# Guitaricet/relora

Measured on NVIDIA H100. Metric: training throughput, llama ReLoRA (tokens/s, whole job, device-timed, max over ranks), higher is better.
Workload: dtype bf16

## Files before the change

relora_b200/csrc/attention.cu:

```cuda
#include <cuda.h>

#include <cstdio>
#include <cstdlib>
#include <mutex>
#include <stdexcept>
#include <string>
#include <unordered_map>

#include "attention.h"
#include "common.cuh"
#include "sm90.cuh"
#include "tensormap.h"

namespace rb {

using namespace sm90;

namespace {

constexpr int BQ = 64;
constexpr int kPanel = 64 * 128;
constexpr int kThreads = 128;
constexpr int kMaxHeadDim = 256;
constexpr float kNegInf = -1e30f;

constexpr int smem_bytes(int nres, int np) { return (nres + 4) * np * kPanel + 1024 + 1024; }
constexpr int dq_out_panels(int np) { return np <= 3 ? np : 2; }
constexpr int dkv_out_panels(int np) { return np <= 2 ? np : 2; }
constexpr int splits(int np, int no) { return (np + no - 1) / no; }

__device__ __forceinline__ float fast_exp2(float x) {
  float y;
  asm("ex2.approx.ftz.f32 %0, %1;" : "=f"(y) : "f"(x));
  return y;
}

__device__ __forceinline__ void frag_to_a(const float (&d)[32], int kk, uint32_t (&a)[4]) {
  a[0] = pack_bf16x2(d[8 * kk + 0], d[8 * kk + 1]);
  a[1] = pack_bf16x2(d[8 * kk + 2], d[8 * kk + 3]);
  a[2] = pack_bf16x2(d[8 * kk + 4], d[8 * kk + 5]);
  a[3] = pack_bf16x2(d[8 * kk + 6], d[8 * kk + 7]);
}
template <int NSTEPS>
__device__ __forceinline__ void mma_steps_kk(float (&d)[32], uint32_t a, uint32_t b) {
#pragma unroll
  for (int ks = 0; ks < NSTEPS; ++ks) {
    const uint32_t ofs = (ks >> 2) * kPanel + (ks & 3) * 32;
    wgmma_bf16_ss_n64<0, 0>(d, desc_kmajor(a + ofs), desc_kmajor(b + ofs));
  }
}
template <int NP>
__device__ __forceinline__ void mma_tiles_kk(float (&d)[32], uint32_t a, uint32_t b, int nks) {
  if constexpr (NP == 1) {
    mma_steps_kk<4>(d, a, b);
  } else {
    switch (nks - 4 * (NP - 1)) {
      case 1: mma_steps_kk<4 * NP - 3>(d, a, b); break;
      case 2: mma_steps_kk<4 * NP - 2>(d, a, b); break;
      case 3: mma_steps_kk<4 * NP - 1>(d, a, b); break;
      default: mma_steps_kk<4 * NP>(d, a, b); break;
    }
  }
}
__device__ __forceinline__ void pack_a(const float (&p)[32], uint32_t (&a)[4][4]) {
#pragma unroll
  for (int kk = 0; kk < 4; ++kk) {
    frag_to_a(p, kk, a[kk]);
    fence_regs(a[kk]);
  }
}
template <int NO, int N = NO>
__device__ __forceinline__ void mma_regs_tile(float (&d)[NO][32], const uint32_t (&a)[4][4], uint32_t t, int nout) {
  if constexpr (N > 1) {
    if (nout < N) return mma_regs_tile<NO, N - 1>(d, a, t, nout);
  }
#pragma unroll
  for (int kk = 0; kk < 4; ++kk) {
#pragma unroll
    for (int j = 0; j < N; ++j) wgmma_bf16_rs_n64<1>(d[j], a[kk], desc_mnmajor(t + j * kPanel + kk * 2048));
  }
}
__device__ __forceinline__ void zero32(float (&d)[32]) {
#pragma unroll
  for (int i = 0; i < 32; ++i) d[i] = 0.f;
}

struct Smem {
  uint8_t* res[2];
  uint8_t* str[2][2];
  uint64_t* res_bar;
  uint64_t* str_bar;
  float* col_lse;
  float* col_delta;
};
template <int NRES, int NP>
__device__ __forceinline__ Smem smem_layout() {
  constexpr int kTile = NP * kPanel;
  extern __shared__ uint8_t smem_raw[];
  uint8_t* s = reinterpret_cast<uint8_t*>((reinterpret_cast<uintptr_t>(smem_raw) + 1023) & ~uintptr_t(1023));
  Smem m;
  m.res[0] = s;
  m.res[1] = s + (NRES - 1) * kTile;
  for (int b = 0; b < 2; ++b)
    for (int o = 0; o < 2; ++o) m.str[b][o] = s + (NRES + 2 * b + o) * kTile;
  m.res_bar = reinterpret_cast<uint64_t*>(s + (NRES + 4) * kTile);
  m.str_bar = m.res_bar + 1;
  m.col_lse = reinterpret_cast<float*>(s + (NRES + 4) * kTile + 64);
  m.col_delta = m.col_lse + 64;
  return m;
}
struct TileSrc {
  const CUtensorMap* map;
  int head;
};
template <int NP>
__device__ __forceinline__ void load_tile(TileSrc s, uint64_t* bar, uint8_t* dst, int row) {
#pragma unroll
  for (int pn = 0; pn < NP; ++pn) tma_load_3d(s.map, bar, dst + pn * kPanel, 64 * pn, s.head, row);
}
template <int NP>
__device__ __forceinline__ void issue_pair(const Smem& m, int buf, TileSrc s0, TileSrc s1, int row) {
  mbar_arrive_expect_tx(&m.str_bar[buf], 2 * NP * kPanel);
  load_tile<NP>(s0, &m.str_bar[buf], m.str[buf][0], row);
  load_tile<NP>(s1, &m.str_bar[buf], m.str[buf][1], row);
}
template <int NRES, int NP>
__device__ __forceinline__ void prologue(const Smem& m, TileSrc r0, TileSrc r1, int res_row, TileSrc s0, TileSrc s1, int row0, int nblk) {
  if (threadIdx.x == 0) {
    mbar_init(m.res_bar, 1);
    mbar_init(&m.str_bar[0], 1);
    mbar_init(&m.str_bar[1], 1);
    fence_barrier_init();
  }
  __syncthreads();
  pdl_wait();
  if (warp_id() == 0) {
    if (elect_one()) {
      mbar_arrive_expect_tx(m.res_bar, NRES * NP * kPanel);
      load_tile<NP>(r0, m.res_bar, m.res[0], res_row);
      if (NRES == 2) load_tile<NP>(r1, m.res_bar, m.res[1], res_row);
      for (int j = 0; j < 2 && j < nblk; ++j) issue_pair<NP>(m, j, s0, s1, row0 + j * BQ);
    }
    __syncwarp();
  }
  mbar_wait(m.res_bar, 0);
}

struct HeadMap {
  int hs, wk, wv, group;
  __device__ __forceinline__ int q(int h) const { return h * hs; }
  __device__ __forceinline__ int k(int kv) const { return kv * hs + wk; }
  __device__ __forceinline__ int v(int kv) const { return kv * hs + wv; }
};
struct FwdArgs {
  bf16* out;
  long long ld_out;
  float* lse;
  int B, T, nh, hd;
  float scale_log2;
  HeadMap hm;
};

template <int NP>
__global__ void __launch_bounds__(kThreads) attn_fwd_kernel(const __grid_constant__ CUtensorMap map_qkv, const FwdArgs p) {
  if (threadIdx.x == 0) pdl_launch_dependents();
  const int nqb = (p.T + BQ - 1) / BQ;
  const int qb = nqb - 1 - blockIdx.x;
  const int h = blockIdx.y, b = blockIdx.z;
  const int q0 = qb * BQ, rowbase = b * p.T;
  const int nkb = qb + 1;
  const int nks = (p.hd + 15) / 16;
  const Smem m = smem_layout<1, NP>();
  const int kv = h / p.hm.group;
  const int hq = p.hm.q(h), hk = p.hm.k(kv), hv = p.hm.v(kv);
  prologue<1, NP>(m, {&map_qkv, hq}, {&map_qkv, hq}, rowbase + q0, {&map_qkv, hk}, {&map_qkv, hv}, rowbase, nkb);
  const uint32_t sq = smem_u32(m.res[0]);
  float o[NP][32], mrow[2] = {kNegInf, kNegInf}, lrow[2] = {0.f, 0.f};
#pragma unroll
  for (int pn = 0; pn < NP; ++pn) zero32(o[pn]);
  const int r_lo = q0 + frag_row(0);
  for (int j = 0; j < nkb; ++j) {
    const int buf = j & 1;
    mbar_wait(&m.str_bar[buf], (j >> 1) & 1);
    float s[32];
    zero32(s);
    wgmma_fence();
    mma_tiles_kk<NP>(s, sq, smem_u32(m.str[buf][0]), nks);
    wgmma_commit();
    wgmma_wait<0>();
    fence_regs(s);
    float mx[2] = {mrow[0], mrow[1]};
#pragma unroll
    for (int i = 0; i < 32; ++i) {
      const int hr = (i >> 1) & 1;
      float v = s[i] * p.scale_log2;
      if (j == qb && j * BQ + frag_col(i) > r_lo + 8 * hr) v = kNegInf;
      s[i] = v;
      mx[hr] = fmaxf(mx[hr], v);
    }
#pragma unroll
    for (int hr = 0; hr < 2; ++hr) {
      mx[hr] = fmaxf(mx[hr], __shfl_xor_sync(0xffffffffu, mx[hr], 1));
      mx[hr] = fmaxf(mx[hr], __shfl_xor_sync(0xffffffffu, mx[hr], 2));
    }
    const float corr[2] = {fast_exp2(mrow[0] - mx[0]), fast_exp2(mrow[1] - mx[1])};
    float ls[2] = {0.f, 0.f};
#pragma unroll
    for (int i = 0; i < 32; ++i) {
      const int hr = (i >> 1) & 1;
      s[i] = fast_exp2(s[i] - mx[hr]);
      ls[hr] += s[i];
#pragma unroll
      for (int pn = 0; pn < NP; ++pn) o[pn][i] *= corr[hr];
    }
#pragma unroll
    for (int hr = 0; hr < 2; ++hr) {
      lrow[hr] = lrow[hr] * corr[hr] + ls[hr];
      mrow[hr] = mx[hr];
    }
    uint32_t pa[4][4];
    pack_a(s, pa);
#pragma unroll
    for (int pn = 0; pn < NP; ++pn) fence_regs(o[pn]);
    wgmma_fence();
    mma_regs_tile<NP>(o, pa, smem_u32(m.str[buf][1]), NP);
    wgmma_commit();
    wgmma_wait<0>();
#pragma unroll
    for (int pn = 0; pn < NP; ++pn) fence_regs(o[pn]);
    __syncthreads();
    if (warp_id() == 0 && j + 2 < nkb) {
      if (elect_one()) issue_pair<NP>(m, buf, {&map_qkv, hk}, {&map_qkv, hv}, rowbase + (j + 2) * BQ);
      __syncwarp();
    }
  }
#pragma unroll
  for (int hr = 0; hr < 2; ++hr) {
    lrow[hr] += __shfl_xor_sync(0xffffffffu, lrow[hr], 1);
    lrow[hr] += __shfl_xor_sync(0xffffffffu, lrow[hr], 2);
  }
#pragma unroll
  for (int pn = 0; pn < NP; ++pn) {
#pragma unroll
    for (int i = 0; i < 32; i += 2) {
      const int hr = (i >> 1) & 1;
      const int q = r_lo + 8 * hr, c = 64 * pn + frag_col(i);
      if (q >= p.T || c >= p.hd) continue;
      const float inv = 1.f / lrow[hr];
      *reinterpret_cast<uint32_t*>(p.out + (long long)(rowbase + q) * p.ld_out + h * p.hd + c) =
          pack_bf16x2(o[pn][i] * inv, o[pn][i + 1] * inv);
    }
  }
  if ((threadIdx.x & 3) == 0) {
#pragma unroll
    for (int hr = 0; hr < 2; ++hr) {
      const int q = r_lo + 8 * hr;
      if (q < p.T) p.lse[((long long)b * p.nh + h) * p.T + q] = mrow[hr] + __log2f(lrow[hr]);
    }
  }
}

__global__ void __launch_bounds__(256) attn_delta_kernel(const bf16* __restrict__ o, long long ld_o, const bf16* __restrict__ dout,
                                                         long long ld_do, float* __restrict__ delta, int B, int T, int nh, int hd) {
  pdl_wait();
  pdl_launch_dependents();
  const long long total = (long long)B * T * nh;
  for (long long i = blockIdx.x * (long long)blockDim.x + threadIdx.x; i < total; i += (long long)gridDim.x * blockDim.x) {
    const int h = int(i % nh);
    const long long row = i / nh;
    const bf16* a = o + row * ld_o + h * hd;
    const bf16* g = dout + row * ld_do + h * hd;
    float acc = 0.f;
    for (int q = 0; q < hd; q += 8) {
      float x[8], y[8];
      unpack8(*reinterpret_cast<const uint4*>(a + q), x);
      unpack8(*reinterpret_cast<const uint4*>(g + q), y);
#pragma unroll
      for (int j = 0; j < 8; ++j) acc += x[j] * y[j];
    }
    const long long bb = row / T, t = row % T;
    delta[(bb * nh + h) * T + t] = acc;
  }
}

struct BwdArgs {
  const float* lse;
  const float* delta;
  bf16* dqkv;
  long long ld_dqkv;
  int B, T, nh, hd;
  float scale, scale_log2;
  HeadMap hm;
};

__device__ __forceinline__ void store_rows(bf16* base, long long ld, int row0, int rows_valid, int col_ofs, int hd, const float (&d)[32], float sc) {
#pragma unroll
  for (int i = 0; i < 32; i += 2) {
    const int r = frag_row(i), c = frag_col(i);
    if (row0 + r >= rows_valid || c >= hd) continue;
    *reinterpret_cast<uint32_t*>(base + (long long)row0 * ld + (long long)r * ld + col_ofs + c) = pack_bf16x2(d[i] * sc, d[i + 1] * sc);
  }
}
template <int NO>
__device__ __forceinline__ void store_panels(bf16* base, long long ld, int row0, int rows_valid, int col_ofs, int hd, int pn0, int nout,
                                             const float (&d)[NO][32], float sc) {
#pragma unroll
  for (int j = 0; j < NO; ++j)
    if (j < nout) store_rows(base, ld, row0, rows_valid, col_ofs + 64 * (pn0 + j), hd - 64 * (pn0 + j), d[j], sc);
}

template <int NP>
__global__ void __launch_bounds__(kThreads) attn_bwd_dq_kernel(const __grid_constant__ CUtensorMap map_qkv,
                                                               const __grid_constant__ CUtensorMap map_do, const BwdArgs p) {
  constexpr int NO = dq_out_panels(NP), NSPLIT = splits(NP, dq_out_panels(NP));
  if (threadIdx.x == 0) pdl_launch_dependents();
  const int nqb = (p.T + BQ - 1) / BQ;
  const int qb = nqb - 1 - blockIdx.x / NSPLIT;
  const int pn0 = (blockIdx.x % NSPLIT) * NO;
  const int nout = NP % NO == 0 ? NO : min(NO, NP - pn0);
  const int h = blockIdx.y, b = blockIdx.z;
  const int q0 = qb * BQ, rowbase = b * p.T;
  const int nkb = qb + 1;
  const int nks = (p.hd + 15) / 16;
  const Smem m = smem_layout<2, NP>();
  const int kv = h / p.hm.group;
  const int hq = p.hm.q(h), hk = p.hm.k(kv), hv = p.hm.v(kv);
  prologue<2, NP>(m, {&map_qkv, hq}, {&map_do, h}, rowbase + q0, {&map_qkv, hk}, {&map_qkv, hv}, rowbase, nkb);
  const long long bh = (long long)b * p.nh + h;
  const int r_lo = q0 + frag_row(0);
  float lse[2], dlt[2];
#pragma unroll
  for (int hr = 0; hr < 2; ++hr) {
    const int q = min(r_lo + 8 * hr, p.T - 1);
    lse[hr] = p.lse[bh * p.T + q];
    dlt[hr] = p.delta[bh * p.T + q];
  }
  float dq[NO][32];
#pragma unroll
  for (int j = 0; j < NO; ++j) zero32(dq[j]);
  for (int j = 0; j < nkb; ++j) {
    const int buf = j & 1;
    mbar_wait(&m.str_bar[buf], (j >> 1) & 1);
    float s[32], dp[32];
    zero32(s);
    zero32(dp);
    wgmma_fence();
    mma_tiles_kk<NP>(s, smem_u32(m.res[0]), smem_u32(m.str[buf][0]), nks);
    mma_tiles_kk<NP>(dp, smem_u32(m.res[1]), smem_u32(m.str[buf][1]), nks);
    wgmma_commit();
    wgmma_wait<0>();
    fence_regs(s);
    fence_regs(dp);
#pragma unroll
    for (int i = 0; i < 32; ++i) {
      const int hr = (i >> 1) & 1;
      const bool ok = !(j == qb && j * BQ + frag_col(i) > r_lo + 8 * hr);
      const float pr = ok ? fast_exp2(s[i] * p.scale_log2 - lse[hr]) : 0.f;
      s[i] = pr * (dp[i] - dlt[hr]);
    }
    uint32_t pa[4][4];
    pack_a(s, pa);
    wgmma_fence();
    mma_regs_tile<NO>(dq, pa, smem_u32(m.str[buf][0]) + pn0 * kPanel, nout);
    wgmma_commit();
    wgmma_wait<0>();
#pragma unroll
    for (int jo = 0; jo < NO; ++jo) fence_regs(dq[jo]);
    __syncthreads();
    if (warp_id() == 0 && j + 2 < nkb) {
      if (elect_one()) issue_pair<NP>(m, buf, {&map_qkv, hk}, {&map_qkv, hv}, rowbase + (j + 2) * BQ);
      __syncwarp();
    }
  }
  store_panels<NO>(p.dqkv + (long long)rowbase * p.ld_dqkv, p.ld_dqkv, q0, p.T, hq * p.hd, p.hd, pn0, nout, dq, p.scale);
}

template <int NP>
__global__ void __launch_bounds__(kThreads) attn_bwd_dkv_kernel(const __grid_constant__ CUtensorMap map_qkv,
                                                                const __grid_constant__ CUtensorMap map_do, const BwdArgs p) {
  constexpr int NO = dkv_out_panels(NP), NSPLIT = splits(NP, dkv_out_panels(NP));
  if (threadIdx.x == 0) pdl_launch_dependents();
  const int nkb = (p.T + BQ - 1) / BQ;
  const int kb = blockIdx.x / NSPLIT;
  const int pn0 = (blockIdx.x % NSPLIT) * NO;
  const int nout = NP % NO == 0 ? NO : min(NO, NP - pn0);
  const int kv = blockIdx.y, b = blockIdx.z;
  const int k0 = kb * BQ, rowbase = b * p.T;
  const int nblk = nkb - kb;
  const int nks = (p.hd + 15) / 16;
  const Smem m = smem_layout<2, NP>();
  const int h0 = kv * p.hm.group;
  prologue<2, NP>(m, {&map_qkv, p.hm.k(kv)}, {&map_qkv, p.hm.v(kv)}, rowbase + k0, {&map_qkv, p.hm.q(h0)}, {&map_do, h0}, rowbase + k0, nblk);
  if (nblk == 1 && p.hm.group > 1 && warp_id() == 0) {
    if (elect_one()) issue_pair<NP>(m, 1, {&map_qkv, p.hm.q(h0 + 1)}, {&map_do, h0 + 1}, rowbase + k0);
    __syncwarp();
  }
  const int key_lo = k0 + frag_row(0);
  float dk[NO][32], dv[NO][32];
#pragma unroll
  for (int j = 0; j < NO; ++j) {
    zero32(dk[j]);
    zero32(dv[j]);
  }
  int hg = h0, qs = k0;
  for (int jj = 0; hg < ((int)blockIdx.y + 1) * p.hm.group; ++jj) {
    const int buf = jj & 1;
    const long long bh = (long long)b * p.nh + hg;
    if (threadIdx.x < BQ) {
      const int qc = min(qs + (int)threadIdx.x, p.T - 1);
      m.col_lse[threadIdx.x] = p.lse[bh * p.T + qc];
      m.col_delta[threadIdx.x] = p.delta[bh * p.T + qc];
    }
    __syncthreads();
    mbar_wait(&m.str_bar[buf], (jj >> 1) & 1);
    float st[32], dpt[32];
    zero32(st);
    zero32(dpt);
    wgmma_fence();
    mma_tiles_kk<NP>(st, smem_u32(m.res[0]), smem_u32(m.str[buf][0]), nks);
    mma_tiles_kk<NP>(dpt, smem_u32(m.res[1]), smem_u32(m.str[buf][1]), nks);
    wgmma_commit();
    wgmma_wait<0>();
    fence_regs(st);
    fence_regs(dpt);
#pragma unroll
    for (int i = 0; i < 32; ++i) {
      const int q = qs + frag_col(i), key = key_lo + 8 * ((i >> 1) & 1);
      const bool ok = q < p.T && key <= q;
      const float pr = ok ? fast_exp2(st[i] * p.scale_log2 - m.col_lse[frag_col(i)]) : 0.f;
      dpt[i] = pr * (dpt[i] - m.col_delta[frag_col(i)]);
      st[i] = pr;
    }
    uint32_t pa[4][4], dsa[4][4];
    pack_a(st, pa);
    pack_a(dpt, dsa);
    wgmma_fence();
    mma_regs_tile<NO>(dv, pa, smem_u32(m.str[buf][1]) + pn0 * kPanel, nout);
    mma_regs_tile<NO>(dk, dsa, smem_u32(m.str[buf][0]) + pn0 * kPanel, nout);
    wgmma_commit();
    wgmma_wait<0>();
#pragma unroll
    for (int j = 0; j < NO; ++j) {
      fence_regs(dv[j]);
      fence_regs(dk[j]);
    }
    __syncthreads();
    if (warp_id() == 0) {
      int h2 = hg, q2 = qs + 2 * BQ;
      while (q2 >= p.T) {
        q2 -= nkb * BQ - k0;
        ++h2;
      }
      if (h2 < ((int)blockIdx.y + 1) * p.hm.group) {
        if (elect_one()) issue_pair<NP>(m, buf, {&map_qkv, p.hm.q(h2)}, {&map_do, h2}, rowbase + q2);
        __syncwarp();
      }
    }
    qs += BQ;
    if (qs >= p.T) {
      qs = k0;
      ++hg;
    }
  }
  bf16* base = p.dqkv + (long long)rowbase * p.ld_dqkv;
  store_panels<NO>(base, p.ld_dqkv, k0, p.T, p.hm.k(blockIdx.y) * p.hd, p.hd, pn0, nout, dk, p.scale);
  store_panels<NO>(base, p.ld_dqkv, k0, p.T, p.hm.v(blockIdx.y) * p.hd, p.hd, pn0, nout, dv, 1.0f);
}

struct HeadMapKey {
  const void* ptr;
  long long ld, rows;
  int hd, heads;
  bool operator==(const HeadMapKey& o) const { return ptr == o.ptr && ld == o.ld && rows == o.rows && hd == o.hd && heads == o.heads; }
};
struct HeadMapHash {
  size_t operator()(const HeadMapKey& k) const {
    size_t h = reinterpret_cast<size_t>(k.ptr);
    h ^= std::hash<long long>()(k.ld * 1315423911ll + k.rows) + 0x9e3779b97f4a7c15ull + (h << 6) + (h >> 2);
    h ^= std::hash<long long>()(((long long)k.hd << 32) | (unsigned)k.heads) + 0x9e3779b97f4a7c15ull + (h << 6) + (h >> 2);
    return h;
  }
};
std::unordered_map<HeadMapKey, CUtensorMap, HeadMapHash> g_head_maps;
std::mutex g_head_maps_mu;

CUtensorMap head_map(const void* ptr, long long ld, long long rows, int hd, int heads) {
  HeadMapKey key{ptr, ld, rows, hd, heads};
  {
    std::lock_guard<std::mutex> lk(g_head_maps_mu);
    auto it = g_head_maps.find(key);
    if (it != g_head_maps.end()) return it->second;
  }
  CUtensorMap m = make_map_3d_bf16(ptr, hd, heads, rows, hd, ld, 64, 1, 64);
  std::lock_guard<std::mutex> lk(g_head_maps_mu);
  if (g_head_maps.size() > 4096) g_head_maps.clear();
  g_head_maps.emplace(key, m);
  return m;
}

void check_shape(int B, int T, int nh, int nkv, int hd, bool interleaved) {
  if (B <= 0 || T <= 0 || nh <= 0) throw std::runtime_error("attention: empty problem");
  if (hd <= 0 || hd % 8 != 0 || hd > kMaxHeadDim)
    throw std::runtime_error("attention: head_dim must be a multiple of 8 and <= 256, got " + std::to_string(hd));
  if (nkv <= 0 || nh % nkv != 0)
    throw std::runtime_error("attention: nh (" + std::to_string(nh) + ") must be a multiple of nkv (" + std::to_string(nkv) + ")");
  if (interleaved && nkv != nh) throw std::runtime_error("attention: the interleaved qkv layout has no grouped-query form (nkv must equal nh)");
}

HeadMap head_map_of(int nh, int nkv, bool interleaved) {
  return interleaved ? HeadMap{3, 1, 2, 1} : HeadMap{1, nh, nh + nkv, nh / nkv};
}

template <int NP>
void fwd_np(const AttnDesc& d, const CUtensorMap& map, cudaStream_t stream) {
  constexpr int smem = smem_bytes(1, NP);
  static const bool configured =
      (check(cudaFuncSetAttribute(attn_fwd_kernel<NP>, cudaFuncAttributeMaxDynamicSharedMemorySize, smem), "cudaFuncSetAttribute(attn_fwd)"), true);
  (void)configured;
  FwdArgs p;
  p.out = reinterpret_cast<bf16*>(d.out); p.ld_out = d.ld_out; p.lse = d.lse;
  p.B = d.B; p.T = d.T; p.nh = d.nh; p.hd = d.hd;
  p.scale_log2 = d.scale * 1.4426950408889634f;
  p.hm = head_map_of(d.nh, d.nkv, d.interleaved);
  const dim3 grid((unsigned)((d.T + BQ - 1) / BQ), (unsigned)d.nh, (unsigned)d.B);
  launch_k(attn_fwd_kernel<NP>, grid, kThreads, smem, stream, map, p);
  RB_CHECK_LAUNCH("attn_fwd_kernel");
}

template <int NP>
void bwd_np(const AttnBwdDesc& d, const CUtensorMap& map_qkv, const CUtensorMap& map_do, cudaStream_t stream) {
  constexpr int smem = smem_bytes(2, NP);
  static const bool configured =
      (check(cudaFuncSetAttribute(attn_bwd_dq_kernel<NP>, cudaFuncAttributeMaxDynamicSharedMemorySize, smem), "cudaFuncSetAttribute(attn_dq)"),
       check(cudaFuncSetAttribute(attn_bwd_dkv_kernel<NP>, cudaFuncAttributeMaxDynamicSharedMemorySize, smem), "cudaFuncSetAttribute(attn_dkv)"),
       true);
  (void)configured;
  BwdArgs p;
  p.lse = d.lse; p.delta = d.delta; p.dqkv = reinterpret_cast<bf16*>(d.dqkv); p.ld_dqkv = d.ld_dqkv;
  p.B = d.B; p.T = d.T; p.nh = d.nh; p.hd = d.hd;
  p.scale = d.scale; p.scale_log2 = d.scale * 1.4426950408889634f;
  p.hm = head_map_of(d.nh, d.nkv, d.interleaved);
  const unsigned nblk = (unsigned)((d.T + BQ - 1) / BQ);
  const dim3 grid_dkv(nblk * splits(NP, dkv_out_panels(NP)), (unsigned)d.nkv, (unsigned)d.B);
  launch_k(attn_bwd_dkv_kernel<NP>, grid_dkv, kThreads, smem, stream, map_qkv, map_do, p);
  RB_CHECK_LAUNCH("attn_bwd_dkv_kernel");
  const dim3 grid_dq(nblk * splits(NP, dq_out_panels(NP)), (unsigned)d.nh, (unsigned)d.B);
  launch_k(attn_bwd_dq_kernel<NP>, grid_dq, kThreads, smem, stream, map_qkv, map_do, p);
  RB_CHECK_LAUNCH("attn_bwd_dq_kernel");
}

int panels(int hd) { return (hd + 63) / 64; }

}

void attention_fwd(const AttnDesc& d, cudaStream_t stream) {
  check_shape(d.B, d.T, d.nh, d.nkv, d.hd, d.interleaved);
  const long long rows = (long long)d.B * d.T;
  CUtensorMap map = head_map(d.qkv, d.ld_qkv, rows, d.hd, d.nh + 2 * d.nkv);
  switch (panels(d.hd)) {
    case 1: fwd_np<1>(d, map, stream); break;
    case 2: fwd_np<2>(d, map, stream); break;
    case 3: fwd_np<3>(d, map, stream); break;
    default: fwd_np<4>(d, map, stream); break;
  }
}

void attention_bwd(const AttnBwdDesc& d, cudaStream_t stream) {
  check_shape(d.B, d.T, d.nh, d.nkv, d.hd, d.interleaved);
  const long long rows = (long long)d.B * d.T;
  CUtensorMap map_qkv = head_map(d.qkv, d.ld_qkv, rows, d.hd, d.nh + 2 * d.nkv);
  CUtensorMap map_do = head_map(d.dout, d.ld_dout, rows, d.hd, d.nh);
  {
    const long long total = rows * d.nh;
    const int grid = (int)std::min<long long>((total + 255) / 256, (long long)num_sms() * 8);
    launch_k(attn_delta_kernel, grid, 256, 0, stream, reinterpret_cast<const bf16*>(d.out), d.ld_out, reinterpret_cast<const bf16*>(d.dout),
             d.ld_dout, d.delta, d.B, d.T, d.nh, d.hd);
    RB_CHECK_LAUNCH("attn_delta_kernel");
  }
  switch (panels(d.hd)) {
    case 1: bwd_np<1>(d, map_qkv, map_do, stream); break;
    case 2: bwd_np<2>(d, map_qkv, map_do, stream); break;
    case 3: bwd_np<3>(d, map_qkv, map_do, stream); break;
    default: bwd_np<4>(d, map_qkv, map_do, stream); break;
  }
}

int attention_smem_bytes(int hd) { return smem_bytes(2, panels(hd)); }

long long attention_ds_pitch(int T) { return ((long long)T + 63) / 64 * 64; }
long long attention_ds_workspace_elems(int B, int T, int nh) {
  const long long Tp = attention_ds_pitch(T);
  return (long long)B * nh * Tp * Tp;
}

}
```

Measured before the change: 215,100.

## Prefetch dKV backward LSE/delta stats via cp.async into double-buffered smem

The dK/dV backward kernel used to load per-query LSE and delta values with plain global loads plus a __syncthreads at the top of every iteration. Those loads now go through cp.async into a double-buffered stats region and are tied to the same mbarrier as the TMA tile loads. The barrier arrival count is raised to cover the 32 cp.async arrivals from warp 0. This removes a blocking global load and a full-block barrier from each loop step, at the cost of a little extra shared memory and more complex barrier accounting.

```diff
diff --git a/relora_b200/csrc/attention.cu b/relora_b200/csrc/attention.cu
--- a/relora_b200/csrc/attention.cu
+++ b/relora_b200/csrc/attention.cu
@@ -25,6 +25,7 @@
 constexpr float kNegInf = -1e30f;
 
 constexpr int smem_bytes(int nres, int np) { return (nres + 4) * np * kPanel + 1024 + 1024; }
+constexpr int kStatsBytes = 2 * 128 * 4;
 constexpr int dq_out_panels(int np) { return np <= 3 ? np : 2; }
 constexpr int dkv_out_panels(int np) { return np <= 2 ? np : 2; }
 constexpr int splits(int np, int no) { return (np + no - 1) / no; }
@@ -90,8 +91,7 @@
   uint8_t* str[2][2];
   uint64_t* res_bar;
   uint64_t* str_bar;
-  float* col_lse;
-  float* col_delta;
+  float* stats;
 };
 template <int NRES, int NP>
 __device__ __forceinline__ Smem smem_layout() {
@@ -105,8 +105,7 @@
     for (int o = 0; o < 2; ++o) m.str[b][o] = s + (NRES + 2 * b + o) * kTile;
   m.res_bar = reinterpret_cast<uint64_t*>(s + (NRES + 4) * kTile);
   m.str_bar = m.res_bar + 1;
-  m.col_lse = reinterpret_cast<float*>(s + (NRES + 4) * kTile + 64);
-  m.col_delta = m.col_lse + 64;
+  m.stats = reinterpret_cast<float*>(s + (NRES + 4) * kTile + 1024);
   return m;
 }
 struct TileSrc {
@@ -375,6 +374,36 @@
   store_panels<NO>(p.dqkv + (long long)rowbase * p.ld_dqkv, p.ld_dqkv, q0, p.T, hq * p.hd, p.hd, pn0, nout, dq, p.scale);
 }
 
+__device__ __forceinline__ void cp_async_4(void* smem_dst, const void* gmem_src) {
+  asm volatile("cp.async.ca.shared.global [%0], [%1], 4;" ::"r"(smem_u32(smem_dst)), "l"(gmem_src) : "memory");
+}
+__device__ __forceinline__ void cp_async_arrive_noinc(uint64_t* bar) {
+  asm volatile("cp.async.mbarrier.arrive.noinc.shared::cta.b64 [%0];" ::"r"(smem_u32(bar)) : "memory");
+}
+template <int NP>
+__device__ __forceinline__ void dkv_issue(const Smem& m, int buf, const CUtensorMap* map_qkv, const CUtensorMap* map_do,
+                                          const BwdArgs& p, int b, int h, int q) {
+  const long long base = ((long long)b * p.nh + h) * p.T;
+  float* st = m.stats + 128 * buf;
+  for (int c = lane_id(); c < BQ; c += 32) {
+    const int qc = min(q + c, p.T - 1);
+    cp_async_4(st + c, p.lse + base + qc);
+    cp_async_4(st + 64 + c, p.delta + base + qc);
+  }
+  cp_async_arrive_noinc(&m.str_bar[buf]);
+  if (elect_one()) issue_pair<NP>(m, buf, {map_qkv, p.hm.q(h)}, {map_do, h}, b * p.T + q);
+  __syncwarp();
+}
+__device__ __forceinline__ void dkv_scores(float (&st)[32], float (&dpt)[32], const float* stats, float scale_log2, int qs, int key_lo, int T) {
+#pragma unroll
+  for (int i = 0; i < 32; ++i) {
+    const int c = frag_col(i);
+    const bool ok = qs + c < T && key_lo + 8 * ((i >> 1) & 1) <= qs + c;
+    const float pr = ok ? fast_exp2(st[i] * scale_log2 - stats[c]) : 0.f;
+    dpt[i] = pr * (dpt[i] - stats[64 + c]);
+    st[i] = pr;
+  }
+}
 template <int NP>
 __global__ void __launch_bounds__(kThreads) attn_bwd_dkv_kernel(const __grid_constant__ CUtensorMap map_qkv,
                                                                 const __grid_constant__ CUtensorMap map_do, const BwdArgs p) {
@@ -390,11 +419,31 @@
   const int nks = (p.hd + 15) / 16;
   const Smem m = smem_layout<2, NP>();
   const int h0 = kv * p.hm.group;
-  prologue<2, NP>(m, {&map_qkv, p.hm.k(kv)}, {&map_qkv, p.hm.v(kv)}, rowbase + k0, {&map_qkv, p.hm.q(h0)}, {&map_do, h0}, rowbase + k0, nblk);
-  if (nblk == 1 && p.hm.group > 1 && warp_id() == 0) {
-    if (elect_one()) issue_pair<NP>(m, 1, {&map_qkv, p.hm.q(h0 + 1)}, {&map_do, h0 + 1}, rowbase + k0);
+  if (threadIdx.x == 0) {
+    mbar_init(m.res_bar, 1);
+    mbar_init(&m.str_bar[0], 1 + 32);
+    mbar_init(&m.str_bar[1], 1 + 32);
+    fence_barrier_init();
+  }
+  __syncthreads();
+  pdl_wait();
+  if (warp_id() == 0) {
+    if (elect_one()) {
+      mbar_arrive_expect_tx(m.res_bar, 2 * NP * kPanel);
+      load_tile<NP>({&map_qkv, p.hm.k(kv)}, m.res_bar, m.res[0], rowbase + k0);
+      load_tile<NP>({&map_qkv, p.hm.v(kv)}, m.res_bar, m.res[1], rowbase + k0);
+    }
     __syncwarp();
-  }
+    for (int j = 0, h = h0, q = k0; j < 2 && h < h0 + p.hm.group; ++j) {
+      dkv_issue<NP>(m, j, &map_qkv, &map_do, p, b, h, q);
+      q += BQ;
+      if (q >= p.T) {
+        q = k0;
+        ++h;
+      }
+    }
+  }
+  mbar_wait(m.res_bar, 0);
   const int key_lo = k0 + frag_row(0);
   float dk[NO][32], dv[NO][32];
 #pragma unroll
@@ -405,13 +454,6 @@
   int hg = h0, qs = k0;
   for (int jj = 0; hg < ((int)blockIdx.y + 1) * p.hm.group; ++jj) {
     const int buf = jj & 1;
-    const long long bh = (long long)b * p.nh + hg;
-    if (threadIdx.x < BQ) {
-      const int qc = min(qs + (int)threadIdx.x, p.T - 1);
-      m.col_lse[threadIdx.x] = p.lse[bh * p.T + qc];
-      m.col_delta[threadIdx.x] = p.delta[bh * p.T + qc];
-    }
-    __syncthreads();
     mbar_wait(&m.str_bar[buf], (jj >> 1) & 1);
     float st[32], dpt[32];
     zero32(st);
@@ -423,14 +465,7 @@
     wgmma_wait<0>();
     fence_regs(st);
     fence_regs(dpt);
-#pragma unroll
-    for (int i = 0; i < 32; ++i) {
-      const int q = qs + frag_col(i), key = key_lo + 8 * ((i >> 1) & 1);
-      const bool ok = q < p.T && key <= q;
-      const float pr = ok ? fast_exp2(st[i] * p.scale_log2 - m.col_lse[frag_col(i)]) : 0.f;
-      dpt[i] = pr * (dpt[i] - m.col_delta[frag_col(i)]);
-      st[i] = pr;
-    }
+    dkv_scores(st, dpt, m.stats + 128 * buf, p.scale_log2, qs, key_lo, p.T);
     uint32_t pa[4][4], dsa[4][4];
     pack_a(st, pa);
     pack_a(dpt, dsa);
@@ -451,10 +486,7 @@
         q2 -= nkb * BQ - k0;
         ++h2;
       }
-      if (h2 < ((int)blockIdx.y + 1) * p.hm.group) {
-        if (elect_one()) issue_pair<NP>(m, buf, {&map_qkv, p.hm.q(h2)}, {&map_do, h2}, rowbase + q2);
-        __syncwarp();
-      }
+      if (h2 < ((int)blockIdx.y + 1) * p.hm.group) dkv_issue<NP>(m, buf, &map_qkv, &map_do, p, b, h2, q2);
     }
     qs += BQ;
     if (qs >= p.T) {
@@ -532,7 +564,7 @@
   constexpr int smem = smem_bytes(2, NP);
   static const bool configured =
       (check(cudaFuncSetAttribute(attn_bwd_dq_kernel<NP>, cudaFuncAttributeMaxDynamicSharedMemorySize, smem), "cudaFuncSetAttribute(attn_dq)"),
-       check(cudaFuncSetAttribute(attn_bwd_dkv_kernel<NP>, cudaFuncAttributeMaxDynamicSharedMemorySize, smem), "cudaFuncSetAttribute(attn_dkv)"),
+       check(cudaFuncSetAttribute(attn_bwd_dkv_kernel<NP>, cudaFuncAttributeMaxDynamicSharedMemorySize, smem + kStatsBytes), "cudaFuncSetAttribute(attn_dkv)"),
        true);
   (void)configured;
   BwdArgs p;
@@ -542,7 +574,7 @@
   p.hm = head_map_of(d.nh, d.nkv, d.interleaved);
   const unsigned nblk = (unsigned)((d.T + BQ - 1) / BQ);
   const dim3 grid_dkv(nblk * splits(NP, dkv_out_panels(NP)), (unsigned)d.nkv, (unsigned)d.B);
-  launch_k(attn_bwd_dkv_kernel<NP>, grid_dkv, kThreads, smem, stream, map_qkv, map_do, p);
+  launch_k(attn_bwd_dkv_kernel<NP>, grid_dkv, kThreads, smem + kStatsBytes, stream, map_qkv, map_do, p);
   RB_CHECK_LAUNCH("attn_bwd_dkv_kernel");
   const dim3 grid_dq(nblk * splits(NP, dq_out_panels(NP)), (unsigned)d.nh, (unsigned)d.B);
   launch_k(attn_bwd_dq_kernel<NP>, grid_dq, kThreads, smem, stream, map_qkv, map_do, p);
@@ -585,7 +617,7 @@
   }
 }
 
-int attention_smem_bytes(int hd) { return smem_bytes(2, panels(hd)); }
+int attention_smem_bytes(int hd) { return smem_bytes(2, panels(hd)) + kStatsBytes; }
 
 long long attention_ds_pitch(int T) { return ((long long)T + 63) / 64 * 64; }
 long long attention_ds_workspace_elems(int B, int T, int nh) {
```

Result: no change. 216,400 (median of 6 runs) (+0.6%).
